# dexsuite/dex-retargeting

Hardware: AMD Instinct MI355X
Metric: retargeted frames/sec (whole node) + max |Δqpos| vs ref, Allegro vector batch 65536 (higher is better)
Workload: dtype f32; 1 GPU; Allegro right hand, VectorOptimizer, 65536 frames/GPU, human-keypoint refs (fixture frame b mod 621 + 2 mm noi; batch_per_gpu=65536, n_opt=16, n_ref=4, collective=none

## Files before the change

### dex_retargeting_amd/csrc/dexr_api.hip

```cpp
#include <hip/hip_runtime.h>

#include <cstdarg>
#include <cstddef>
#include <cstdio>
#include <cstdlib>
#include <atomic>
#include <cstring>
#include <mutex>
#include <new>
#include <string>
#include <vector>

#include "dexr.h"
#include "dexr_gen.hpp"
#include "dexr_hostctx.hpp"
#include "dexr_launch.hpp"

namespace {

thread_local std::string g_err;

int fail(int code, const char* fmt, ...) {
  char buf[512];
  va_list ap;
// ... 159 lines not shown

}
size_t dexr_fleet_ws_ints();
size_t dexr_fleet_order_ws_ints(int64_t B);
hipError_t dexr_fleet_dexpilot_order_launch(int64_t B, const float* kpts, const uint32_t* state, const int32_t* perm, const int32_t* seg,
                                            int n_kp, const int32_t* h_task, const int32_t* h_origin, int F, float project_dist,
                                            float escape_dist, int32_t* xws, const int32_t** out_perm, const int32_t** out_seg,
                                            hipStream_t st);
hipError_t dexr_dexpilot_order_launch(int64_t B, const float* kpts, const float* ref, const uint32_t* state, int n_kp, int n_ref,
                                      const int32_t* h_task, const int32_t* h_origin, int F, float project_dist, float escape_dist,
                                      int32_t* key, int32_t* ws, hipStream_t st);
namespace {

bool wide_modchol_rule(const dexr_model* m) {
  return m->wide_mimic && (m->tune.pivot_rule > 0 || (m->tune.pivot_rule < 0 && m->h.kind == DEXR_KIND_DEXPILOT));
}

int launch_wide_once(const dexr_model* m, dexr::KernelParams kp, hipStream_t st, bool f64 = false) {
  const bool modchol = f64 ? wide_modchol_rule(m) : m->wide_modchol;
  const size_t per_wave = f64 ? (m->wide_mimic ? (modchol ? dexr::wide_lds_per_wave_d_mc_16() : dexr::wide_lds_per_wave_d_m_16())
                                               : (m->wbucket == 16 ? dexr::wide_lds_per_wave_d_16() : m->wbucket == 24 ? dexr::wide_lds_per_wave_d_24() : 0))
                              : m->wide_mimic ? dexr::wide_lds_per_wave_m_16() : dexr::wide_lds_per_wave(m->wbucket);
  if (per_wave == 0) return fail(DEXR_ERR_UNSUPPORTED, "no float64 sixteen-lane kernel for bucket %d", m->wbucket);
  if (kp.kpts && kp.n_kp > 85) return fail(DEXR_ERR_UNSUPPORTED, "the sixteen-lane kernel takes at most 85 keypoints per frame (%d)", kp.n_kp);
  int wpb = 4;
  while (wpb > 1 && per_wave * wpb > (f64 ? 160 : 80) * 1024) wpb >>= 1;
  const int64_t sprint_max = m->tune.sprint_max_batch < 0 ? 2048 : m->tune.sprint_max_batch;
  const bool sprint = !f64 && kp.B <= sprint_max && kp.n_comp == 1;
  const int fpw = sprint ? 1 : 4;
  {
    const bool ladder = sprint && m->tune.sprint_ladder != 0;
    const float mu_on[4] = {0.03f, 0.3f, 3.f, 30.f};
    for (int r = 0; r < 4; ++r) kp.sprint_mu[r] = ladder ? mu_on[r] : 1.f;
    if (ladder || f64) kp.blind_tol = 0.f;
  }
  const int64_t tiles = (kp.B + fpw - 1) / fpw;
  const int occ = f64 ? 1 : sprint ? ((!m->wide_mimic && m->wbucket > 24) ? 1 : 2) : ((!m->wide_mimic && m->wbucket == 16) ? 3 : 2);
  int64_t resident = (int64_t)m->n_cu * 4 * occ;
  if (m->tune.resident_waves > 0) resident = m->tune.resident_waves;
  int64_t per_comp = (resident + kp.n_comp - 1) / kp.n_comp;
  if (per_comp > tiles) per_comp = tiles;
  const int64_t waves = per_comp * kp.n_comp;
  const int64_t blocks = (waves + wpb - 1) / wpb;
  if (blocks > 0x7fffffffLL) return fail(DEXR_ERR_INVALID, "batch too large for one launch");
  kp.q0 = (uint32_t)(per_comp * fpw);
  { const int rc = take_queue(m, kp, st, (int64_t)kp.q0 < kp.B); if (rc != DEXR_OK) return rc; }
#ifdef DEXR_WIDE_PROF
  static double* wprof = nullptr;
  if (!wprof) (void)hipMalloc((void**)&wprof, 12 * sizeof(double));
  (void)hipMemsetAsync(wprof, 0, 12 * sizeof(double), st);
  kp.g64out = wprof;
#endif
  dexr::wide_launch_fn fn = f64 ? (m->wide_mimic ? (modchol ? dexr::launch_wide_d_mc_16 : dexr::launch_wide_d_m_16)
                                                 : m->wbucket == 16 ? dexr::launch_wide_d_16 : m->wbucket == 24 ? dexr::launch_wide_d_24 : nullptr)
                          : m->wide_mimic ? (sprint ? (m->wide_modchol ? dexr::launch_wide_s_mc_16 : dexr::launch_wide_s_m_16)
                                                    : (m->wide_modchol ? dexr::launch_wide_mc_16 : dexr::launch_wide_m_16))
                            : sprint      ? dexr::find_wide_sprint_launcher(m->wbucket)
                                          : dexr::find_wide_launcher(m->wbucket);
  if (!fn) return fail(DEXR_ERR_UNSUPPORTED, "no sixteen-lane kernel for bucket %d", m->wbucket);
  hipError_t e = fn(kp, m->d_wide, dim3((unsigned)blocks), dim3(64 * wpb), per_wave * wpb, st);
  if (e != hipSuccess) return fail(DEXR_ERR_HIP, "kernel launch failed: %s", hipGetErrorString(e));
#ifdef DEXR_WIDE_PROF
  {
    double h[12];
    (void)hipStreamSynchronize(st);
    (void)hipMemcpy(h, wprof, sizeof(h), hipMemcpyDeviceToHost);
    const char* names[9] = {"hand-out", "fk", "terms", "term loop", "2nd order", "accept/active set", "factor+solve", "step", "retire"};
    fprintf(stderr, "[wprof] B=%lld passes(wave 0)=%.0f cycles per pass:", (long long)kp.B, h[11]);
    for (int i = 0; i < 9; ++i) fprintf(stderr, " %s %.0f |", names[i], h[11] > 0 ? h[i] / h[11] : 0.0);
    fprintf(stderr, "\n");
  }
#endif
  return DEXR_OK;
}

size_t lpt_slot_bytes(int64_t B) {
  const size_t b = (size_t)B;
  return b * sizeof(int32_t) + (dexr_fleet_ws_ints() + b) * sizeof(int32_t);
}
int lpt_slot_grow(dexr_model::LptSlot& sl, size_t bytes) {
  if (sl.bytes >= bytes) return DEXR_OK;
  if (sl.buf) {
    if (sl.done) HIP_TRY(hipEventSynchronize(sl.done));
    HIP_TRY(hipFree(sl.buf));
    sl.buf = nullptr;
    sl.bytes = 0;
  }
  HIP_TRY(hipMalloc(&sl.buf, bytes));
  sl.bytes = bytes;
  return DEXR_OK;
}

int launch_wide(const dexr_model* m, dexr::KernelParams kp, hipStream_t st, bool f64 = false) {
  const int want = m->tune.longest_first;
  const bool plain = !kp.perm && !kp.bucket && kp.T == 0 && kp.n_comp == 1;
  const bool by_state = plain && kp.kind == DEXR_KIND_DEXPILOT &&
                        (want == 2 || (want < 0 && kp.n_opt >= 9 && kp.B >= 4 * (int64_t)m->n_cu * 4 * 2 * 4));
  if (!by_state) return launch_wide_once(m, kp, st, f64);
  hipStreamCaptureStatus cap = hipStreamCaptureStatusNone;
  if (hipStreamIsCapturing(st, &cap) != hipSuccess || cap != hipStreamCaptureStatusNone)
    return launch_wide_once(m, kp, st, f64);
  const size_t bytes = lpt_slot_bytes(kp.B);
  dexr_model::LptSlot& sl = m->lpt[m->lnext.fetch_add(1u) % dexr_model::LSLOTS];
  if (!sl.done) HIP_TRY(hipEventCreateWithFlags(&sl.done, hipEventDisableTiming));
  else HIP_TRY(hipStreamWaitEvent(st, sl.done, 0));
  { const int rc = lpt_slot_grow(sl, bytes); if (rc != DEXR_OK) return rc; }
  int32_t* key = static_cast<int32_t*>(sl.buf);
  int32_t* ws = key + kp.B;
  hipError_t e = dexr_dexpilot_order_launch(kp.B, kp.kpts, kp.ref, kp.state, kp.n_kp, kp.n_ref, kp.h_task, kp.h_origin, kp.num_fingers,
                                            kp.project_dist, kp.escape_dist, key, ws, st);
  if (e != hipSuccess) return fail(DEXR_ERR_HIP, "ordering kernels failed: %s", hipGetErrorString(e));
  kp.perm = ws + dexr_fleet_ws_ints();
  const int rc = launch_wide_once(m, kp, st, f64);
  HIP_TRY(hipEventRecord(sl.done, st));
  return rc;
}

bool build_wide_tables(dexr_model* m) {
  m->wide_tabs.clear();
  m->wide_mimic = m->has_mimic;
  m->wbucket = m->bucket < 16 ? 16 : m->bucket;
  if (m->bucket < 8 || m->h.kind == DEXR_KIND_FKONLY) return false;
  if (m->has_mimic && (m->max_vars > 16 || m->max_joints > 32)) return false;
  for (const dexr_comp_table& c : m->comps) {
    dexr::WideTable w;
    std::memset(&w, 0, sizeof(w));
    std::memset(w.chain, 0xFF, sizeof(w.chain));
    const int nj = c.n_joint;
    if (c.n_term > 16 || c.n_frame > 16) return false;
    int parent[DEXR_MAXJ], slot_owner[DEXR_NSLOT + 1];
    bool has_child[DEXR_MAXJ];
    for (int s = 0; s <= DEXR_NSLOT; ++s) slot_owner[s] = -1;
    for (int k = 0; k < nj; ++k) {
      has_child[k] = false;
      if (c.src_kind[k] != DEXR_SRC_OPT && c.src_kind[k] != DEXR_SRC_FIXED && c.src_kind[k] != DEXR_SRC_MIMIC) return false;
      const int rs = c.restore[k];
      if (rs == -2) parent[k] = -1;
      else if (rs >= 0) { if (rs > DEXR_NSLOT) return false; parent[k] = slot_owner[rs]; }
      else parent[k] = k - 1;
      if (c.save[k] >= 0) { if (c.save[k] > DEXR_NSLOT) return false; slot_owner[c.save[k]] = k; }
    }
    for (int k = 0; k < nj; ++k)
      if (parent[k] >= 0) has_child[parent[k]] = true;
    bool published[DEXR_MAXJ];
    for (int k = 0; k < nj; ++k) {
      published[k] = false;
      uint32_t anc = 0;
      for (int j = k; j >= 0; j = parent[j])
        if (c.jtype[j] == DEXR_JOINT_REVOLUTE) anc |= 1u << j;
      w.anc_rev[k] = anc;
    }
    int n_chain = 0, depth = 0;
    for (int k = 0; k < nj; ++k) {
      if (has_child[k]) continue;
      if (n_chain == 16) return false;
      int path[DEXR_MAXJ], len = 0;
      for (int j = k; j >= 0; j = parent[j]) path[len++] = j;
      if (len > 16) return false;
      for (int s = 0; s < len; ++s) {
        const int j = path[len - 1 - s];
        w.chain[n_chain][s] = (uint8_t)(j | (published[j] ? 0 : 0x80));
        published[j] = true;
      }
      if (len > depth) depth = len;
      ++n_chain;
    }
    w.n_chain = n_chain;
    w.depth = depth;
    std::memset(w.fam, 0xFF, sizeof(w.fam));
    if (m->has_mimic) {
      int fam_n[16] = {0};
      for (int v = 0; v < c.n_var; ++v) w.fam[v][fam_n[v]++] = (uint8_t)c.var_joint[v];
      for (int k = 0; k < nj; ++k) {
        const int v = c.var[k];
        if (v < 0 || c.var_joint[v] == k) continue;
        if (fam_n[v] == 3) return false;
        w.fam[v][fam_n[v]++] = (uint8_t)k;
      }
      for (int v = 0; v < c.n_var; ++v) w.fam_max = fam_n[v] > w.fam_max ? fam_n[v] : w.fam_max;
      struct PairRec { int lane; uint32_t word; };
      std::vector<PairRec> recs;
      for (int k = 0; k < nj; ++k) {
        if (c.var[k] < 0) continue;
        for (int j = k; j >= 0; j = parent[j]) {
          if (c.jtype[j] != DEXR_JOINT_REVOLUTE || c.var[j] < 0) continue;
          const int vk = c.var[k], vj = c.var[j];
          const int vhi = vk > vj ? vk : vj, vlo = vk > vj ? vj : vk;
          const int i = vhi >> 2, jj = vlo >> 2;
          const uint32_t dbl = (j != k && vk == vj) ? 1u : 0u;
          recs.push_back({(vhi & 3) * 4 + (vlo & 3), (uint32_t)k | ((uint32_t)j << 5) | ((uint32_t)(i * (i + 1) / 2 + jj) << 10) | (dbl << 14)});
        }
      }
      if (recs.size() > 128) return false;
      int n = 0;
      for (int ln = 0; ln < 16; ++ln) {
        w.pair_off[ln] = (uint8_t)n;
        for (const PairRec& r : recs)
          if (r.lane == ln) w.pair[n++] = r.word;
        const int cnt = n - w.pair_off[ln];
        if (cnt > w.pair_max) w.pair_max = cnt;
      }
      w.pair_off[16] = (uint8_t)n;
    }
    m->wide_tabs.push_back(w);
  }
  return true;
}

#ifndef DEXR_GEN_LAM_JUMP
#define DEXR_GEN_LAM_JUMP 0.03f
#endif
int launch_gen_model(const dexr_model* m, int mode, dexr::KernelParams kp, hipStream_t st, const dexr::GenVjp* vj = nullptr) {
  const size_t lds = dexr::gen_lds_bytes(m->gen_tab);
  if (lds > 160 * 1024) return fail(DEXR_ERR_UNSUPPORTED, "model needs %zu B of LDS per frame", lds);
  int64_t per_cu = (int64_t)((160 * 1024) / lds);
  per_cu = per_cu < 1 ? 1 : (per_cu > 8 ? 8 : per_cu);
  int64_t blocks = (int64_t)m->n_cu * per_cu;
  if (blocks > kp.B) blocks = kp.B;
#ifdef DEXR_GEN_PROF
  static double* gprof = nullptr;
  if (mode == dexr::MODE_SOLVE) {
    if (!gprof) (void)hipMalloc((void**)&gprof, 12 * sizeof(double));
    (void)hipMemsetAsync(gprof, 0, 12 * sizeof(double), st);
    kp.g64out = gprof;
  }
#endif
  kp.lam_jump = m->lam_jump_user >= 0.f ? m->lam_jump_user : DEXR_GEN_LAM_JUMP;
  hipError_t e = dexr::launch_gen(mode, kp, m->gen_tab, dim3((unsigned)blocks), lds, st, vj);
  if (e != hipSuccess) return fail(DEXR_ERR_HIP, "kernel launch failed: %s", hipGetErrorString(e));
#ifdef DEXR_GEN_PROF
  if (mode == dexr::MODE_SOLVE) {
    double h[12];
    (void)hipStreamSynchronize(st);
    (void)hipMemcpy(h, gprof, sizeof(h), hipMemcpyDeviceToHost);
    const char* names[8] = {"kinematics", "terms", "term loop", "2nd order", "active set + matrix", "factorisation", "solves", "step + pred"};
    fprintf(stderr, "[gprof] B=%lld blocks=%lld lds=%zu passes(block 0)=%.0f cycles per pass:", (long long)kp.B, (long long)blocks, lds, h[11]);
    for (int i = 0; i < 8; ++i) fprintf(stderr, " %s %.0f |", names[i], h[11] > 0 ? h[i] / h[11] : 0.0);
    fprintf(stderr, "\n");
  }
#endif
  return DEXR_OK;
}

#ifndef DEXR_RED_SMALL_BATCH
#define DEXR_RED_SMALL_BATCH 16384
#endif
bool wide_f64_selected(const dexr_model* m) { return !m->gen && m->tune.kernel_f64 == DEXR_KERNEL_WIDE && m->wide_ok; }

int launch(const dexr_model* m, int mode, int f64, dexr::KernelParams kp, hipStream_t st, bool f64_request = false) {
  if (kp.B <= 0) return DEXR_OK;
  if (m->gen) return launch_gen_model(m, mode, kp, st);
  if (mode == dexr::MODE_SOLVE && f64 && f64_request && wide_f64_selected(m) && !kp.perm && !kp.bucket) {
    kp.lam_jump = m->lam_jump_user >= 0.f ? m->lam_jump_user : wide_modchol_rule(m) ? family_lam_jump(m, FAM_REGISTER) : 1.0f;
    kp.lam_fastdec = family_lam_fastdec(m, FAM_WIDE);
    return launch_wide(m, kp, st, true);
  }
  const bool ext = kp.perm != nullptr || kp.bucket != nullptr || kp.T > 0 || kp.ld != kp.n_opt;
  if (mode == dexr::MODE_SOLVE && !f64 && selected_family(m) != FAM_REGISTER) {
    Family fam = selected_family(m);
    if (fam == FAM_RED && m->wide_ok && m->tune.kernel == DEXR_KERNEL_AUTO && kp.B <= DEXR_RED_SMALL_BATCH) fam = FAM_WIDE;
    kp.lam_jump = family_lam_jump(m, fam);
    kp.lam_fastdec = family_lam_fastdec(m, fam);
    return fam == FAM_RED ? launch_red(m, kp, st) : launch_wide(m, kp, st);
  }
  kp.lam_jump = family_lam_jump(m, FAM_REGISTER);
  if (m->bucket == 32 && mode == dexr::MODE_SOLVE) f64 = 1;
  const size_t real_sz = f64 ? 8 : 4;
  const bool tip_kernel = m->tip && m->chain && m->bucket == 4 && mode == dexr::MODE_SOLVE;
  const size_t per_wave = 64 * real_sz * (size_t)(3 * m->lds_frames + 4 * m->lds_terms + (tip_kernel ? 1 : 0) + ((tip_kernel && f64) ? 18 : 0));
#ifndef DEXR_WPB
#define DEXR_WPB 4
#endif
  int wpb = DEXR_WPB;
#ifndef DEXR_TIP_WPB_BIG
#define DEXR_TIP_WPB_BIG 8
#endif
  if (tip_kernel && !f64 && (kp.B + 63) / 64 * kp.n_comp >= 4096) wpb = DEXR_TIP_WPB_BIG;
  const size_t block_lds_cap = (tip_kernel && f64) ? 64 * 1024 : 48 * 1024;
  while (wpb > 1 && per_wave * wpb > block_lds_cap) wpb >>= 1;
  if (per_wave > 64 * 1024) return fail(DEXR_ERR_UNSUPPORTED, "component needs %zu B of LDS per wave", per_wave);
  const int64_t tiles = (kp.B + 63) / 64;
  int64_t waves = tiles * kp.n_comp;
  if (mode == dexr::MODE_SOLVE && m->bucket <= 8) {
    int occ = m->chain ? 4 : (m->bucket <= 4 ? 3 : 2);
    if (f64) occ = tip_kernel ? 2 : 1;
    if (m->tune.persist_occ > 0) occ = m->tune.persist_occ;
    const int64_t resident = (int64_t)m->n_cu * 4 * occ;
    const int64_t per_comp = (resident + kp.n_comp - 1) / kp.n_comp;
    const int64_t persist_from = m->tune.persist_from;
    kp.qchunk = 0;
    if (tiles >= persist_from * per_comp) {
      waves = per_comp * kp.n_comp;
      kp.q0 = (uint32_t)(per_comp * 64);
      kp.qchunk = m->tune.qchunk > 0 ? (uint32_t)m->tune.qchunk : 256u;
    }
    if (kp.qchunk) {
      const int rc = take_queue(m, kp, st);
      if (rc != DEXR_OK) return rc;
    }
  }
  const int64_t blocks = (waves + wpb - 1) / wpb;
  if (blocks > 0x7fffffffLL) return fail(DEXR_ERR_INVALID, "batch too large for one launch");
  dexr::launch_fn fn = dexr::find_launcher(m->bucket, f64, mode, m->chain, ext, m->tip);
#if !defined(DEXR_SMALL_PROF) && !defined(DEXR_WAVE_TRACE)
  if (tip_kernel && !f64 && !ext && kp.qchunk == 0 && kp.T == 0 && !kp.fval && !kp.x0 && !kp.qout64 && m->tune.kernel != DEXR_KERNEL_REGISTER_CHAIN)
    fn = dexr::launch_tip32;
#endif
  if (!fn) return fail(DEXR_ERR_UNSUPPORTED, "no kernel for bucket %d / f64=%d / mode=%d", m->bucket, f64, mode);
#ifdef DEXR_SMALL_PROF
  static double* sprof = nullptr;
  const bool sprof_on = mode == dexr::MODE_SOLVE && m->bucket <= 8;
  if (sprof_on) {
    if (!sprof) (void)hipMalloc((void**)&sprof, 12 * sizeof(double));
    (void)hipMemsetAsync(sprof, 0, 12 * sizeof(double), st);
    kp.g64out = sprof;
  }
#endif
#ifdef DEXR_WAVE_TRACE
  static double* wtrace = nullptr;
  static size_t wtrace_cap = 0;
  const bool wtrace_on = mode == dexr::MODE_SOLVE && m->bucket <= 8;
  const size_t wtrace_n = (size_t)blocks * wpb * 24;
  if (wtrace_on) {
    if (wtrace_n > wtrace_cap) {
      if (wtrace) (void)hipFree(wtrace);
      (void)hipMalloc((void**)&wtrace, wtrace_n * sizeof(double));
      wtrace_cap = wtrace_n;
    }
    (void)hipMemsetAsync(wtrace, 0, wtrace_n * sizeof(double), st);
    kp.g64out = wtrace;
  }
#endif
  hipError_t e = fn(kp, dim3((unsigned)blocks), dim3(64 * wpb), per_wave * wpb, st);
  if (e != hipSuccess) return fail(DEXR_ERR_HIP, "kernel launch failed: %s", hipGetErrorString(e));
#ifdef DEXR_WAVE_TRACE
  if (wtrace_on) {
    std::vector<double> h(wtrace_n);
    (void)hipStreamSynchronize(st);
    (void)hipMemcpy(h.data(), wtrace, wtrace_n * sizeof(double), hipMemcpyDeviceToHost);
    if (FILE* f = fopen("/tmp/dexr_wave_trace.bin", "wb")) {
      fwrite(h.data(), sizeof(double), wtrace_n, f);
      fclose(f);
    }
  }
#endif
#ifdef DEXR_SMALL_PROF
  if (sprof_on) {
    double h[12];
    (void)hipStreamSynchronize(st);
    (void)hipMemcpy(h, sprof, sizeof(h), hipMemcpyDeviceToHost);
    const char* names[6] = {"hand-out", "step", "fk", "residuals", "accept", "retire"};
    fprintf(stderr, "[sprof] B=%lld passes(wave 0)=%.0f cycles per pass:", (long long)kp.B, h[11]);
    for (int i = 0; i < 6; ++i) fprintf(stderr, " %s %.0f |", names[i], h[11] > 0 ? h[i] / h[11] : 0.0);
    fprintf(stderr, "\n");
  }
#endif
  return DEXR_OK;
}

void default_tuning(dexr_model* m) {
  dexr_tuning& t = m->tune;
  std::memset(&t, 0, sizeof(t));
  t.struct_size = (uint32_t)sizeof(dexr_tuning);
  t.kernel = DEXR_KERNEL_AUTO;
  t.chain = 1;
  t.persist_occ = 0;
  t.persist_from = 8;
  t.qchunk = 256;
  t.resident_waves = 0;
  t.max_blind = 8;
  t.stall_from = 2;
  t.stall_ratio = 0.9f;
  t.stall_cap = 20.f;
  t.lam_jump = m->bucket <= 8 ? 3.0f : 0.3f;
  t.lam_fastdec = m->bucket <= 8 ? 0.1f : 0.f;
  t.lam_recover = 0.f;
  t.floor_scale = 1e-12f;
  t.step_cap = 0.3f;
  t.blind_tol_scale = m->bucket <= 8 ? 100.f : 10.f;
  t.pivot_rule = -1;
  t.longest_first = -1;
  t.fork_streams = -1;
  t.sprint_max_batch = -1;
  t.sprint_ladder = -1;
  t.tail_passes = -1;
  t.kernel_f64 = DEXR_KERNEL_AUTO;
}

int create_generic(const dexr_model_header& h, const char* body, size_t nbytes, dexr_model** out) {
  if (h.version != DEXR_TABLE_VERSION) return fail(DEXR_ERR_INVALID, "table version %u, library expects %u", h.version, DEXR_TABLE_VERSION);
  if (nbytes < sizeof(dexr_gen_header)) return fail(DEXR_ERR_INVALID, "blob shorter than the generic-table header");
  dexr_gen_header gh;
  std::memcpy(&gh, body, sizeof(gh));
  if (gh.magic != DEXR_GEN_MAGIC) return fail(DEXR_ERR_INVALID, "n_comp = 0 but no generic table follows the header");
  const int nj = gh.n_joint, nf = gh.n_frame, nt = gh.n_term, nv = gh.n_var, nfam = gh.n_fam;
  if (nj < 0 || nj > DEXR_GEN_MAXJ || nf < 1 || nf > DEXR_GEN_MAXJ || nt < 1 || nt > DEXR_GEN_MAXJ || nv < 0 || nv > nj ||
      nfam < nv || nfam > nj || gh.max_depth < 0 || gh.max_depth > nj)
    return fail(DEXR_ERR_INVALID, "generic table sizes out of range (%d joints, %d frames, %d terms, %d variables)", nj, nf, nt, nv);
  if (h.kind != DEXR_KIND_FKONLY && nv != h.n_opt) return fail(DEXR_ERR_INVALID, "generic table has %d variables, header n_opt = %d", nv, h.n_opt);
  if (nt != h.n_ref) return fail(DEXR_ERR_INVALID, "generic table has %d terms, header n_ref = %d", nt, h.n_ref);
  if (h.kind == DEXR_KIND_DEXPILOT) {
    const int F = h.num_fingers;
    if (F < 2 || F > 8) return fail(DEXR_ERR_INVALID, "DexPilot needs 2..8 fingers (32 projection bits), got %d", F);
    if (h.n_ref != F * (F - 1) / 2 + F) return fail(DEXR_ERR_INVALID, "DexPilot n_ref=%d does not match %d fingers", h.n_ref, F);
  }
  auto pad2 = [](size_t n) { return (n + 1) & ~(size_t)1; };
  const size_t n_f64 = (size_t)nj * 12 + (size_t)nj * 3 + 2 * (size_t)nj + 2 * (size_t)nv + (size_t)nf * 3;
  const size_t n_u64 = (size_t)nf + nj;
  const size_t i32_sizes[14] = {(size_t)nj, (size_t)nj, (size_t)nj, (size_t)nj, (size_t)nj, (size_t)nv, (size_t)nv + 1,
                                (size_t)nfam, (size_t)nf, (size_t)nt, (size_t)nt, (size_t)nt, (size_t)nt, (size_t)nt};
  size_t n_i32 = 0;
  for (size_t v : i32_sizes) n_i32 += pad2(v);
  const size_t want = sizeof(gh) + 8 * (n_f64 + n_u64) + 4 * n_i32;
  if (nbytes != want) return fail(DEXR_ERR_INVALID, "generic table is %zu B, its header implies %zu B", nbytes, want);
  const char* p = body + sizeof(gh);
  const double* f64 = reinterpret_cast<const double*>(p);
  const unsigned long long* u64 = reinterpret_cast<const unsigned long long*>(p + 8 * n_f64);
  const int32_t* i32 = reinterpret_cast<const int32_t*>(p + 8 * (n_f64 + n_u64));
  const int32_t* arr[14];
  {
    size_t o = 0;
    for (int i = 0; i < 14; ++i) {
      arr[i] = i32 + o;
      o += pad2(i32_sizes[i]);
    }
  }
  const int32_t *jtype = arr[0], *parent = arr[1], *depth = arr[2], *src_idx = arr[3], *var = arr[4], *var_api = arr[5],
                *fam_off = arr[6], *fam = arr[7], *frame_joint = arr[8], *term_task = arr[9], *term_origin = arr[10],
                *term_ref = arr[11], *row_ho = arr[12], *row_ht = arr[13];
  for (int k = 0; k < nj; ++k) {
    const bool bad = (jtype[k] != DEXR_JOINT_REVOLUTE && jtype[k] != DEXR_JOINT_PRISMATIC) || parent[k] < -1 || parent[k] >= k ||
                     depth[k] != (parent[k] < 0 ? 0 : depth[parent[k]] + 1) || depth[k] > gh.max_depth || var[k] < -1 || var[k] >= nv ||
                     (var[k] < 0 && h.kind != DEXR_KIND_FKONLY && (src_idx[k] < 0 || src_idx[k] >= h.n_fixed)) ||
                     (h.kind == DEXR_KIND_FKONLY && (src_idx[k] < 0 || src_idx[k] >= h.n_q));
    if (bad) return fail(DEXR_ERR_INVALID, "generic table: joint record %d malformed", k);
  }
  for (int v = 0; v < nv; ++v) {
    if (var_api[v] < 0 || var_api[v] >= h.n_opt || fam_off[v] < 0 || fam_off[v] > fam_off[v + 1] || fam_off[v + 1] > nfam)
      return fail(DEXR_ERR_INVALID, "generic table: variable record %d malformed", v);
    for (int e = fam_off[v]; e < fam_off[v + 1]; ++e)
      if (fam[e] < 0 || fam[e] >= nj || var[fam[e]] != v) return fail(DEXR_ERR_INVALID, "generic table: family of variable %d malformed", v);
  }
  for (int f = 0; f < nf; ++f)
    if (frame_joint[f] < -1 || frame_joint[f] >= nj) return fail(DEXR_ERR_INVALID, "generic table: frame record %d malformed", f);
  std::vector<bool> seen((size_t)nt, false);
  for (int t = 0; t < nt; ++t) {
    const bool bad = term_task[t] < 0 || term_task[t] >= nf || term_origin[t] < -1 || term_origin[t] >= nf || term_ref[t] < 0 ||
                     term_ref[t] >= nt || seen[(size_t)term_ref[t]] ||
                     (gh.has_keypoint_map && (row_ht[t] < 0 || row_ht[t] >= h.n_keypoints || row_ho[t] < -1 || row_ho[t] >= h.n_keypoints));
    if (bad) return fail(DEXR_ERR_INVALID, "generic table: term record %d malformed", t);
    seen[(size_t)term_ref[t]] = true;
  }
  dexr_model* m = new (std::nothrow) dexr_model();
  if (!m) return fail(DEXR_ERR_INVALID, "out of host memory");
  m->h = h;
  m->gen = true;
  m->bucket = 0;
  m->max_joints = nj;
  m->max_vars = nv;
  default_tuning(m);
  m->has_mimic = nfam > nv;
  const size_t payload = nbytes - sizeof(gh);
  hipError_t e = hipMalloc(&m->d_gen, payload ? payload : 8);
  if (e == hipSuccess) e = hipMemcpy(m->d_gen, p, payload, hipMemcpyHostToDevice);
  if (e == hipSuccess) {
    int dev = 0, cus = 0;
    if (hipGetDevice(&dev) == hipSuccess &&
        hipDeviceGetAttribute(&cus, hipDeviceAttributeMultiprocessorCount, dev) == hipSuccess && cus > 0)
      m->n_cu = cus;
  }
  if (e != hipSuccess) {
    if (m->d_gen) (void)hipFree(m->d_gen);
    delete m;
    return fail(DEXR_ERR_HIP, "uploading tables failed: %s", hipGetErrorString(e));
  }
  const char* d = static_cast<const char*>(m->d_gen);
  const double* df = reinterpret_cast<const double*>(d);
  dexr::GenTab& g = m->gen_tab;
  g.nj = nj; g.nf = nf; g.nt = nt; g.nv = nv; g.nfam = nfam; g.max_depth = gh.max_depth; g.has_kp = gh.has_keypoint_map;
  g.X = df;
  g.axis = g.X + (size_t)nj * 12;
  g.jmul = g.axis + (size_t)nj * 3;
  g.joff = g.jmul + nj;
  g.lo = g.joff + nj;
  g.hi = g.lo + nv;
  g.frame_off = g.hi + nv;
  g.frame_anc = reinterpret_cast<const unsigned long long*>(d + 8 * n_f64);
  g.joint_anc = g.frame_anc + nf;
  const int32_t* di = reinterpret_cast<const int32_t*>(d + 8 * (n_f64 + n_u64));
  const int32_t** dst[14] = {&g.jtype, &g.parent, &g.depth, &g.src_idx, &g.var, &g.var_api, &g.fam_off, &g.fam, &g.frame_joint,
                             &g.term_task, &g.term_origin, &g.term_ref, &g.row_ho, &g.row_ht};
  {
    size_t o = 0;
    for (int i = 0; i < 14; ++i) {
      *dst[i] = di + o;
      o += pad2(i32_sizes[i]);
    }
  }
  (void)u64;
  (void)f64;
  *out = m;
  return DEXR_OK;
}

bool wide_wins_small(const dexr_model* m) {
  return m->bucket == 8 && m->h.n_comp == 1 && (m->h.kind == DEXR_KIND_POSITION || m->h.kind == DEXR_KIND_DEXPILOT);
}

void select_kernels(dexr_model* m) {
  const dexr_model_header& h = m->h;
  const int want = m->tune.kernel;
  m->red_nv = m->max_vars <= 8 ? 8 : (m->max_vars <= 16 ? 16 : 0);
  const size_t red_lds = (size_t)64 * (4 * 6 * (size_t)m->max_joints + 8 * 3 * (size_t)m->lds_frames);
  const bool red_ok = m->red_nv > 0 && h.kind != DEXR_KIND_FKONLY && m->max_slot < 2 && red_lds <= 160 * 1024 && m->max_joints > 0;
  const bool red_wins = m->has_mimic && m->bucket >= 16;
  m->red = red_ok && (want == DEXR_KERNEL_REDUCED || (want == DEXR_KERNEL_AUTO && red_wins));
  m->wide = m->wide_ok && (want == DEXR_KERNEL_WIDE || (want == DEXR_KERNEL_AUTO && (m->bucket >= 16 || wide_wins_small(m))));
  if (m->wide && m->has_mimic && want == DEXR_KERNEL_AUTO && h.kind == DEXR_KIND_VECTOR && red_ok) m->wide = false;
  m->wide_modchol = m->wide && m->wide_mimic && (m->tune.pivot_rule > 0 || (m->tune.pivot_rule < 0 && h.kind == DEXR_KIND_DEXPILOT));
  m->red = m->red && !m->wide;
  m->chain = m->tune.chain != 0 && (h.kind == DEXR_KIND_VECTOR || h.kind == DEXR_KIND_POSITION);
  for (const dexr_comp_table& c : m->comps) {
    if (c.n_joint != m->bucket || c.n_frame > dexr::LocalTab<4>::LF || c.n_term > dexr::LocalTab<4>::LT) m->chain = false;
    for (int k = 0; k < c.n_joint && m->chain; ++k)
      if (c.restore[k] != (k == 0 ? -2 : -1) || c.save[k] != -1 || c.src_kind[k] != DEXR_SRC_OPT ||
          c.jtype[k] != DEXR_JOINT_REVOLUTE)
        m->chain = false;
  }
  if (m->bucket != 4) m->chain = false;
  m->tip = m->chain && m->tune.chain == 1 && h.kind == DEXR_KIND_VECTOR;
  for (size_t ci = 0; ci < m->comps.size() && m->tip; ++ci) {
    const dexr_comp_table& c = m->comps[ci];
    if (c.n_term != 1) { m->tip = false; break; }
    const int ft = c.term_task[0], fo = c.term_origin[0];
    if (ft < 0 || ft >= c.n_frame || fo < 0 || fo >= c.n_frame || c.frame_joint[ft] != 3 || c.frame_joint[fo] != -1) m->tip = false;
    for (int k = 1; k < 4 && m->tip; ++k)
      if (c.api[k] != c.api[0] + k) m->tip = false;
  }
}

void apply_options(const dexr_model* m, dexr::KernelParams& kp, const dexr_solve_options* opt) {
  dexr_solve_options o;
  dexr_default_options(&o);
  if (opt) o = *opt;
  kp.max_iter = o.max_iter > 0 ? o.max_iter : 64;
  kp.tol = o.tol > 0 ? o.tol : 2e-6f;
  kp.lam0 = o.lambda0 > 0 ? o.lambda0 : 1e-4f;
  kp.newton = o.newton;
  kp.max_blind = m->tune.max_blind;
  kp.blind_tol = m->tune.blind_tol_scale * kp.tol;
  kp.stall_from = m->tune.stall_from;
  kp.stall_ratio = m->tune.stall_ratio;
  kp.stall_cap = m->tune.stall_cap;
}

bool polish_wanted(const dexr_model* m, const dexr_solve_options* opt) {
  if (m->gen) return false;
  int polish = opt ? opt->polish : -1;
  if (polish < 0) polish = (m->h.kind == DEXR_KIND_POSITION || m->h.kind == DEXR_KIND_DEXPILOT) ? 24 : 0;
  if (polish == 0 || m->bucket == 32) return false;
  if ((m->red || m->wide) && (opt ? opt->strict : 0) <= 0) return false;
  return true;
}

int polish_launch(const dexr_model* m, dexr::KernelParams kp, const dexr_solve_options* opt, hipStream_t st) {
  if (!polish_wanted(m, opt)) return DEXR_OK;
  int polish = opt ? opt->polish : -1;
  if (polish < 0) polish = 24;
  kp.x0 = kp.qout;
  kp.max_iter = polish;
  kp.tol *= 0.25f;
  kp.blind_tol = 10.f * kp.tol;
  kp.fval = nullptr;
  if (kp.perm) kp.status = nullptr;
  if (kp.status) HIP_TRY(hipMemsetAsync(kp.status, 0, (size_t)kp.B * sizeof(int32_t), st));
  return launch(m, dexr::MODE_SOLVE, 1, kp, st);
}

}

int dexr_prep_launch(int64_t B, const float* kp, const float* op9, float* out, float* rot, hipStream_t st);
size_t dexr_fleet_ws_ints();
hipError_t dexr_fleet_bucket_launch(int n_models, int64_t B, const int32_t* model_id, int32_t* ws, hipStream_t st);
hipError_t dexr_dexpilot_order_launch(int64_t B, const float* kpts, const float* ref, const uint32_t* state, int n_kp, int n_ref,
                                      const int32_t* h_task, const int32_t* h_origin, int F, float project_dist, float escape_dist,
                                      int32_t* key, int32_t* ws, hipStream_t st);
hipError_t dexr_seq_compose_launch(int64_t B, int T, int n_q, int n_opt, int n_fixed, const int32_t* kind,
                                   const int32_t* idx, const double* mult, const double* off, const float* qraw,
                                   const float* fixed, double alpha, int use_filter, int first_frame_initialises,
                                   double* filt, double* out, hipStream_t st);

extern "C" {

const char* dexr_last_error(void) { return g_err.c_str(); }

const char* dexr_version(void) { return "dexr 0.4 (gfx950; table v5 + generic tables)"; }

int dexr_device_count(void) {
  int n = 0;
  if (hipGetDeviceCount(&n) != hipSuccess) return 0;
  return n;
}

void dexr_default_options(dexr_solve_options* opt) {
  if (!opt) return;
  opt->strict = 0;
  opt->max_iter = 64;
// ... 750 lines not shown
```

### dex_retargeting_amd/csrc/dexr_tip_solve.hpp

```cpp
#pragma once
#include "dexr_kernel.hpp"

namespace dexr {

static __device__ __forceinline__ bool tip32_chol(float (&H)[10], const float (&g)[4], float (&d)[4], float pivot_floor) {
  using RT = RealTraits<float, true>;
  constexpr auto hidx = [](int r, int c) constexpr { return r * (r + 1) / 2 + c; };
  bool ok = true;
  float inv[4];
#pragma unroll
  for (int j = 0; j < 4; ++j) {
    float dj = H[hidx(j, j)];
#pragma unroll
    for (int k = 0; k < j; ++k) dj -= H[hidx(j, k)] * H[hidx(j, k)];
    if (!(dj > 1e-6f * pivot_floor)) {
      ok = false;
      dj = fmax(fabs(dj), pivot_floor);
    }
    const float iv = RT::rsqrt(dj);
    inv[j] = iv;
    H[hidx(j, j)] = dj * iv;
#pragma unroll
    for (int i = j + 1; i < 4; ++i) {
      float s = H[hidx(i, j)];
#pragma unroll
      for (int k = 0; k < j; ++k) s -= H[hidx(i, k)] * H[hidx(j, k)];
      H[hidx(i, j)] = s * iv;
    }
  }
#pragma unroll
  for (int i = 0; i < 4; ++i) {
    float s = -g[i];
#pragma unroll
    for (int k = 0; k < i; ++k) s -= H[hidx(i, k)] * d[k];
    d[i] = s * inv[i];
  }
#pragma unroll
  for (int i = 3; i >= 0; --i) {
    float s = d[i];
#pragma unroll
    for (int k = i + 1; k < 4; ++k) s -= H[hidx(k, i)] * d[k];
    d[i] = s * inv[i];
  }
  return ok;
}

__global__ void __launch_bounds__(DEXR_TIP_BLOCK_MAX, DEXR_CHAIN_MINW) dexr_tip32_kernel(const KernelParams kp, const dexr_comp_table* __restrict__ comps) {
  extern __shared__ __align__(16) unsigned char lds_raw[];
  using RT = RealTraits<float, true>;
  constexpr auto hidx = [](int r, int c) constexpr { return r * (r + 1) / 2 + c; };
  float a_delta = kp.norm_delta, a_lam0 = kp.lam0, a_tol = kp.tol, a_blind_tol = kp.blind_tol, a_step_cap = kp.step_cap;
  float a_huber = kp.huber_delta, a_inv_norm = kp.inv_norm, a_lam_fastdec = kp.lam_fastdec, a_lam_jump = kp.lam_jump;
  float a_lam_recover = kp.lam_recover, a_stall_ratio = kp.stall_ratio, a_stall_cap = kp.stall_cap;
  float a_scaling = kp.scaling;
  int a_newton = kp.newton, a_stall_from = kp.stall_from, a_max_blind = kp.max_blind, a_max_iter = kp.max_iter;
  asm volatile(""
               : "+s"(a_delta), "+s"(a_lam0), "+s"(a_tol), "+s"(a_blind_tol), "+s"(a_step_cap), "+s"(a_huber), "+s"(a_inv_norm),
                 "+s"(a_lam_fastdec), "+s"(a_lam_jump), "+s"(a_lam_recover), "+s"(a_stall_ratio), "+s"(a_stall_cap), "+s"(a_newton),
                 "+s"(a_stall_from), "+s"(a_max_blind), "+s"(a_max_iter), "+s"(a_scaling)
               : "s"((int)blockDim.x), "s"(kp.last), "s"(kp.kpts), "s"(kp.ref), "s"(kp.B), "s"(kp.n_comp), "s"(kp.n_opt), "s"(kp.n_kp), "s"(kp.n_ref),
                 "s"(kp.lds_frames), "s"(kp.lds_terms));

  const int lane = threadIdx.x & 63;
  const int wave_in_block = __builtin_amdgcn_readfirstlane(threadIdx.x >> 6);
  const int waves_per_block = blockDim.x >> 6;
  const int64_t wave_global = (int64_t)blockIdx.x * waves_per_block + wave_in_block;
  const int comp = (int)(wave_global % kp.n_comp);
  const int64_t tile = wave_global / kp.n_comp;
  const int64_t nB = kp.B;
  if (tile * 64 >= nB) return;
  const int64_t item = tile * 64 + lane;
  bool has = item < nB;
  const int ld = kp.n_opt;

  const int per_wave = 64 * (3 * kp.lds_frames + 4 * kp.lds_terms + 1);
  float* P = reinterpret_cast<float*>(lds_raw) + (size_t)wave_in_block * per_wave;
  float* T = P + 64 * 3 * kp.lds_frames;
  float* W = T + 64 * 3 * kp.lds_terms;

  const dexr_comp_table& tb = comps[comp];
  TipTabRegs tt;
  TipTabT<float>::Stage st;
  int api0 = tb.api[0];
  int row = tb.term_ref[0], ft = tb.term_task[0], fo = tb.term_origin[0];
  tt.fetch(tb, lane, st);
  tt.hold(st, api0, row, ft, fo);
  const int hrow = row < DEXR_MAXT ? row : DEXR_MAXT - 1;
  int h_t = kp.h_task[hrow], h_o = kp.h_origin[hrow];
  tt.fetch_off(tb, ft, fo, st);
  tt.hold_off(st, h_t, h_o);

  float x[4] = {0.f, 0.f, 0.f, 0.f}, xl[4] = {0.f, 0.f, 0.f, 0.f};
  float fl[4], ra[3], rb[3];
  float tg[3] = {0.f, 0.f, 0.f};
  const bool sub = kp.kpts != nullptr && h_o >= 0;
  if (has) {
    const float* pa = kp.kpts ? kp.kpts + (item * kp.n_kp + h_t) * 3 : kp.ref + (item * kp.n_ref + row) * 3;
    const float* pb = sub ? kp.kpts + (item * kp.n_kp + h_o) * 3 : pa;
#pragma unroll
    for (int k = 0; k < 4; ++k) fl[k] = kp.last[item * ld + api0 + k];
#pragma unroll
    for (int i = 0; i < 3; ++i) {
      ra[i] = pa[i];
      rb[i] = pb[i];
    }
  }

  tt.place<false>(st, fo, W + 64 * kp.lds_terms, lane);

  const float k_delta = a_delta, k_lam0 = a_lam0, k_tol = a_tol, k_blind_tol = a_blind_tol;
  const float k_step_cap = a_step_cap;
  const float tip_beta = a_huber, tip_ibeta = tip_pin(1.f / a_huber);
  const float tip_w = a_inv_norm, tip_nw = tip_pin(a_newton != 0 ? 1.f : 0.f);
  const float k_lam_fastdec = a_lam_fastdec, k_lam_jump = a_lam_jump, k_lam_recover = a_lam_recover;
  const float k_stall_ratio = a_stall_ratio;
  const int k_stall_from = a_stall_from, k_max_blind = a_max_blind, k_max_iter = a_max_iter;
  const float k_2delta = tip_pin(2.f * k_delta), k_10tol = tip_pin(10.f * k_tol);
  const float k_stall_max = tip_pin(a_stall_cap * k_tol);
  const float k_lam_ok = tip_pin(fmax(2.f * k_delta, 10.f * k_lam0)), k_lam_ok_half = tip_pin(0.5f * fmax(2.f * k_delta, 10.f * k_lam0));
  const float k_inf = __builtin_inff();
  const float k_rho_fast = tip_pin(a_lam_fastdec > 0 ? 0.9f : k_inf), k_lam_rec_from = tip_pin(a_lam_recover > 0 ? 10.f * a_lam0 : k_inf);

  if (has) {
    float rv[3];
    if (sub) {
#pragma unroll
      for (int i = 0; i < 3; ++i) rv[i] = ra[i] - rb[i];
    } else {
#pragma unroll
      for (int i = 0; i < 3; ++i) rv[i] = ra[i];
    }
#pragma unroll
    for (int i = 0; i < 3; ++i) tg[i] = rv[i] * a_scaling;
#pragma unroll
    for (int k = 0; k < 4; ++k) {
      xl[k] = fl[k];
      x[k] = RT::clamp(fl[k], tt.lo[k], tt.hi[k]);
    }
  }

  float Hs[10], gs[4], xo[4];
  float F, lam = k_lam0, nu = 2, sprev = 1e30f;
  int my_iters = 0, blind = 0, nrej = 0;

  auto eval = [&](const float (&xe)[4], float (&g)[4], float (&H)[10]) -> float {
    tt.arrived();
    float Ft = tip_eval<float>(tt, xe, tg[0], tg[1], tg[2], tip_beta, tip_ibeta, tip_w, tip_nw, g, H);
#pragma unroll
    for (int k = 0; k < 4; ++k) {
      const float dx = xe[k] - xl[k];
      Ft += k_delta * dx * dx;
      g[k] += k_2delta * dx;
    }
    return Ft;
  };
  auto retire = [&](int status) {
    int l = lane;
    asm volatile("" : "+v"(l));
    const int64_t it = tile * 64 + l;
    bool bad = (status == ST_FALLBACK);
#pragma unroll
    for (int k = 0; k < 4; ++k) bad = bad || !(x[k] == x[k]);
    if (bad) status = ST_FALLBACK;
#pragma unroll
    for (int k = 0; k < 4; ++k) kp.qout[it * ld + api0 + k] = bad ? xl[k] : x[k];
    if (kp.status) atomicMax(&kp.status[it], status);
    if (kp.iters) atomicMax(&kp.iters[it], my_iters);
    has = false;
  };

  tt.prefetch();
  F = eval(x, gs, Hs);
  if (has && !((bool)((int)(F == F) & (int)(fabs(F) < 1e30f)))) retire(ST_FALLBACK);

  while (__any(has)) {
    tt.prefetch();
    float g[4], H[10], d[4];
    bool fr[4];
#pragma unroll
    for (int k = 0; k < 4; ++k) {
      const float gk = gs[k];
      const bool act = (bool)(((int)(x[k] <= tt.lo[k]) & (int)(gk > 0)) | ((int)(x[k] >= tt.hi[k]) & (int)(gk < 0)));
      fr[k] = !act;
      g[k] = !act ? gk : 0.f;
    }
#pragma unroll
    for (int rr = 0; rr < 4; ++rr) {
#pragma unroll
      for (int cc = 0; cc < rr; ++cc) H[hidx(rr, cc)] = (fr[rr] && fr[cc]) ? Hs[hidx(rr, cc)] : 0.f;
      H[hidx(rr, rr)] = fr[rr] ? Hs[hidx(rr, rr)] + k_2delta + lam : 1.f;
    }
    float gm[4];
#pragma unroll
    for (int k = 0; k < 4; ++k) gm[k] = g[k];
    const bool ok = tip32_chol(H, g, d, k_2delta + lam);
    float dmax = 0, gd = 0, dd = d[0] * d[0];
#pragma unroll
    for (int k = 0; k < 4; ++k) {
      dmax = fmax(dmax, fabs(d[k]));
      gd -= gm[k] * d[k];
      if (k > 0) dd = fmaf(d[k], d[k], dd);
    }
    const bool cut = (bool)((int)(k_step_cap > 0) & ((int)(dmax > k_step_cap) | ((int)!ok & (int)(dmax > 0.f))));
    const float alpha = cut ? fmin(RT::div(k_step_cap, dmax), 8.f) : 1.f;
    const float pred = fmaf(alpha * (1.f - 0.5f * alpha), gd, 0.5f * alpha * alpha * lam * dd);
    float smax = 0;
#pragma unroll
    for (int k = 0; k < 4; ++k) {
      xo[k] = x[k];
      const float xt = RT::clamp(x[k] + alpha * d[k], tt.lo[k], tt.hi[k]);
      smax = fmax(smax, fabs(xt - x[k]));
      x[k] = xt;
    }
    const bool last_step = (bool)((int)has & (int)ok & (int)(smax < k_blind_tol) & (int)(lam <= k_lam0) &
                                  ((int)(smax < k_10tol) | (int)(smax < 0.1f * sprev)));

    float Ft = F;
    if (__any(has && !last_step)) Ft = eval(x, g, H);

    bool accept = false, finished = false;
    int status = ST_MAXITER;
    if (has) {
      const bool finite = (bool)((int)(Ft == Ft) & (int)(smax == smax) & (int)(fabs(Ft) < 1e30f));
      if (last_step && finite) {
        accept = true;
        finished = true;
        status = ST_CONVERGED;
        ++my_iters;
        F = Ft;
      } else {
        const float noise = 16.f * RT::eps() * fmax(fabs(F), 2e-3f);
        const bool below_floor = (bool)((int)ok & (int)finite & (int)(pred <= noise) & (int)(smax < 1e-2f));
        accept = (bool)((int)finite & ((int)(Ft <= F) | (int)below_floor));
        ++my_iters;
        if (accept) {
          const float rho = RT::div(F - Ft, fmax(pred, 1e-30f));
          const float t = 2.f * rho - 1.f;
          float shrink = below_floor ? (float)(1.0 / 3.0) : fmax((float)(1.0 / 3.0), 1.f - t * t * t);
          if (rho > k_rho_fast) shrink = (bool)((int)(nrej <= 2) & (int)(lam > k_lam_rec_from)) ? k_lam_recover : k_lam_fastdec;
          lam = fmax(lam * shrink, 1e-9f);
          nu = 2;
          F = Ft;
          const bool stalled = (bool)((int)below_floor & (int)(blind >= k_stall_from) & (int)(smax > k_stall_ratio * sprev) & (int)(smax < k_stall_max));
          blind = below_floor ? blind + 1 : 0;
          sprev = smax;
          if ((bool)(((int)(smax < k_tol) & (int)(lam <= k_lam_ok)) | (int)stalled | (int)(blind >= k_max_blind))) {
            finished = true;
            status = ST_CONVERGED;
          } else if (smax < k_tol) {
            lam = fmax(0.1f * lam, k_lam_ok_half);
          }
        } else {
          ++nrej;
          lam = fmax(lam, 1e-6f) * nu;
          float ds = 0;
#pragma unroll
          for (int k = 0; k < 4; ++k) ds += Hs[hidx(k, k)];
          lam = fmax(lam, k_lam_jump * ds / 4.f);
          nu *= 2;
          if (lam > 1e10f) {
            finished = true;
            status = finite ? ST_CONVERGED : ST_FALLBACK;
          }
          if ((bool)((int)finite & (int)(smax < k_tol))) {
            finished = true;
            status = ST_CONVERGED;
          }
        }
        finished = (bool)((int)finished | (int)(my_iters >= k_max_iter));
      }
    }
#pragma unroll
    for (int k = 0; k < 4; ++k) {
      x[k] = accept ? x[k] : xo[k];
      gs[k] = accept ? g[k] : gs[k];
    }
#pragma unroll
    for (int i = 0; i < 10; ++i) Hs[i] = accept ? H[i] : Hs[i];

    if (finished) retire(status);
  }
}

}
```

Baseline: 1.966 billion frames/s.

## Add wave priority ladder to tip32 solver kernel and wave-trace instrumentation

Adds s_setprio scheduling to the tip32 LM solver kernel. Waves start at high priority and step down over the first iterations, with later blocks decaying faster. A tail boost raises priority again after a few more passes so the last waves finish sooner. The scheme only applies when the grid's wave count falls in a set range. It also adds wave-trace timing instrumentation under a debug macro and lets the tip kernel be used under wave tracing. Priority changes only reorder issue among resident waves, so the effect depends heavily on contention and could also hurt.

```diff
diff --git a/dex_retargeting_amd/csrc/dexr_api.hip b/dex_retargeting_amd/csrc/dexr_api.hip
--- a/dex_retargeting_amd/csrc/dexr_api.hip
+++ b/dex_retargeting_amd/csrc/dexr_api.hip
@@ -485,7 +485,7 @@
   const int64_t blocks = (waves + wpb - 1) / wpb;
   if (blocks > 0x7fffffffLL) return fail(DEXR_ERR_INVALID, "batch too large for one launch");
   dexr::launch_fn fn = dexr::find_launcher(m->bucket, f64, mode, m->chain, ext, m->tip);
-#if !defined(DEXR_SMALL_PROF) && !defined(DEXR_WAVE_TRACE)
+#if !defined(DEXR_SMALL_PROF)
   if (tip_kernel && !f64 && !ext && kp.qchunk == 0 && kp.T == 0 && !kp.fval && !kp.x0 && !kp.qout64 && m->tune.kernel != DEXR_KERNEL_REGISTER_CHAIN)
     fn = dexr::launch_tip32;
 #endif
diff --git a/dex_retargeting_amd/csrc/dexr_tip_solve.hpp b/dex_retargeting_amd/csrc/dexr_tip_solve.hpp
--- a/dex_retargeting_amd/csrc/dexr_tip_solve.hpp
+++ b/dex_retargeting_amd/csrc/dexr_tip_solve.hpp
@@ -45,10 +45,61 @@
   return ok;
 }
 
+#define DEXR_TIP_PRIO_LADDER 1
+#define DEXR_TIP_PRIO_LATE 2
+#define DEXR_TIP_PRIO_PROLOGUE 4
+#define DEXR_TIP_PRIO_TAIL 8
+#ifndef DEXR_TIP_PRIO_TAIL_AFTER
+#define DEXR_TIP_PRIO_TAIL_AFTER 3
+#endif
+#ifndef DEXR_TIP_PRIO
+#define DEXR_TIP_PRIO (DEXR_TIP_PRIO_LADDER | DEXR_TIP_PRIO_LATE | DEXR_TIP_PRIO_TAIL)
+#endif
+#if DEXR_TIP_PRIO & DEXR_TIP_PRIO_TAIL
+#define DEXR_TIP_PRIO_DONE (-2 * DEXR_TIP_PRIO_TAIL_AFTER)
+#else
+#define DEXR_TIP_PRIO_DONE 1
+#endif
+#ifndef DEXR_TIP_PRIO_MIN_WAVES
+#define DEXR_TIP_PRIO_MIN_WAVES 4096
+#endif
+#ifndef DEXR_TIP_PRIO_MAX_WAVES
+#define DEXR_TIP_PRIO_MAX_WAVES 16384
+#endif
+
+#ifdef DEXR_WAVE_TRACE
+#define TIP_WTRACE_PUT(i, v) { if (lane == 0 && wt_o) wt_o[i] = (double)(v); }
+#define TIP_WTRACE_START long long wt_t0 = wall_clock64();
+#define TIP_WTRACE_DECL double* wt_o = kp.g64out ? kp.g64out + (size_t)wave_global * 24 : nullptr; int wt_n = 0; TIP_WTRACE_PUT(0, wt_t0)
+#define TIP_WTRACE_ARRIVED(a, b) { asm volatile("" ::"v"(a), "v"(b)); TIP_WTRACE_PUT(1, wall_clock64()) }
+#define TIP_WTRACE_PASS() { if (wt_n < 16) TIP_WTRACE_PUT(8 + wt_n, wall_clock64()) ++wt_n; }
+#define TIP_WTRACE_FLUSH() { TIP_WTRACE_PUT(2, wall_clock64()) TIP_WTRACE_PUT(3, wt_n) \
+  TIP_WTRACE_PUT(4, __builtin_amdgcn_s_getreg(63492)) TIP_WTRACE_PUT(5, __builtin_amdgcn_s_getreg(63508)) }
+#else
+#define TIP_WTRACE_START
+#define TIP_WTRACE_DECL
+#define TIP_WTRACE_ARRIVED(a, b)
+#define TIP_WTRACE_PASS()
+#define TIP_WTRACE_FLUSH()
+#endif
+
 __global__ void __launch_bounds__(DEXR_TIP_BLOCK_MAX, DEXR_CHAIN_MINW) dexr_tip32_kernel(const KernelParams kp, const dexr_comp_table* __restrict__ comps) {
   extern __shared__ __align__(16) unsigned char lds_raw[];
   using RT = RealTraits<float, true>;
   constexpr auto hidx = [](int r, int c) constexpr { return r * (r + 1) / 2 + c; };
+  TIP_WTRACE_START
+#if DEXR_TIP_PRIO
+  const unsigned prio_waves = gridDim.x * (blockDim.x >> 6);
+  const bool prio_on = prio_waves >= DEXR_TIP_PRIO_MIN_WAVES && prio_waves < DEXR_TIP_PRIO_MAX_WAVES;
+  const bool prio_late = (DEXR_TIP_PRIO & DEXR_TIP_PRIO_LATE) && blockIdx.x * 2u >= gridDim.x;
+  if (prio_on) {
+    if (DEXR_TIP_PRIO & (DEXR_TIP_PRIO_LADDER | DEXR_TIP_PRIO_PROLOGUE)) __builtin_amdgcn_s_setprio(3);
+    else if (prio_late) __builtin_amdgcn_s_setprio(1);
+  }
+#endif
+#if DEXR_TIP_PRIO & DEXR_TIP_PRIO_LADDER
+  int prio_c = prio_on ? (prio_late ? 5 : 6) : DEXR_TIP_PRIO_DONE;
+#endif
   float a_delta = kp.norm_delta, a_lam0 = kp.lam0, a_tol = kp.tol, a_blind_tol = kp.blind_tol, a_step_cap = kp.step_cap;
   float a_huber = kp.huber_delta, a_inv_norm = kp.inv_norm, a_lam_fastdec = kp.lam_fastdec, a_lam_jump = kp.lam_jump;
   float a_lam_recover = kp.lam_recover, a_stall_ratio = kp.stall_ratio, a_stall_cap = kp.stall_cap;
@@ -69,6 +120,7 @@
   const int64_t tile = wave_global / kp.n_comp;
   const int64_t nB = kp.B;
   if (tile * 64 >= nB) return;
+  TIP_WTRACE_DECL
   const int64_t item = tile * 64 + lane;
   bool has = item < nB;
   const int ld = kp.n_opt;
@@ -138,6 +190,7 @@
       x[k] = RT::clamp(fl[k], tt.lo[k], tt.hi[k]);
     }
   }
+  TIP_WTRACE_ARRIVED(x[3], tg[2])
 
   float Hs[10], gs[4], xo[4];
   float F, lam = k_lam0, nu = 2, sprev = 1e30f;
@@ -172,6 +225,12 @@
   tt.prefetch();
   F = eval(x, gs, Hs);
   if (has && !((bool)((int)(F == F) & (int)(fabs(F) < 1e30f)))) retire(ST_FALLBACK);
+#if (DEXR_TIP_PRIO & DEXR_TIP_PRIO_PROLOGUE) && !(DEXR_TIP_PRIO & DEXR_TIP_PRIO_LADDER)
+  if (prio_on) {
+    if (prio_late) __builtin_amdgcn_s_setprio(1);
+    else __builtin_amdgcn_s_setprio(0);
+  }
+#endif
 
   while (__any(has)) {
     tt.prefetch();
@@ -279,7 +338,18 @@
     for (int i = 0; i < 10; ++i) Hs[i] = accept ? H[i] : Hs[i];
 
     if (finished) retire(status);
-  }
+    TIP_WTRACE_PASS()
+#if DEXR_TIP_PRIO & DEXR_TIP_PRIO_LADDER
+    if (prio_c > DEXR_TIP_PRIO_DONE) {
+      prio_c -= 2;
+      if (prio_c >= 3) __builtin_amdgcn_s_setprio(2);
+      else if (prio_c >= 1) __builtin_amdgcn_s_setprio(1);
+      else if (prio_c == 0) __builtin_amdgcn_s_setprio(0);
+      else if (prio_c <= DEXR_TIP_PRIO_DONE) __builtin_amdgcn_s_setprio(3);
+    }
+#endif
+  }
+  TIP_WTRACE_FLUSH()
 }
 
 }
```

After: 2.175 billion frames/s, median of 6. 1.11x the previous value.
